# safe-autonomous-systems/fluidgym

Hardware: NVIDIA B200
Metric: env-steps/sec (solver steps x envs) (higher is better)
Workload: dtype f32

## Files before the change

fluidgym_b200/csrc/piso_b200.cu:

```cuda
#include <cuda_runtime.h>
#include <cooperative_groups.h>
#include <stdint.h>
#include <stdio.h>
#include <stdlib.h>
#include <string.h>
#include <math.h>
#include <new>

#include "fluidgym_b200.h"

namespace cg = cooperative_groups;

static thread_local char g_err[512] = "";
static int set_err(int code, const char *msg, cudaError_t ce = cudaSuccess) {
    if (ce != cudaSuccess) snprintf(g_err, sizeof(g_err), "%s: %s", msg, cudaGetErrorString(ce));
    else snprintf(g_err, sizeof(g_err), "%s", msg);
    return code;
}
extern "C" const char *fgb_last_error(void) { return g_err; }
extern "C" int fgb_version(void) { return 1; }

#define LAUNCH_CHECK(name)                                                       \
    do {                                                                         \
        cudaError_t e_ = cudaGetLastError();                                     \
        if (e_ != cudaSuccess) return set_err(FGB_E_CUDA, name, e_);             \
    } while (0)

typedef fgb_tables Tab;

struct fgb_batch {
    Tab t;
    int B;
    fgb_options opt;
    char *ws;
    size_t ws_bytes;
    float *Coff, *A, *rhs, *ures, *Poff, *Pdiag, *hbya, *div, *pres, *kry;
    float *resid, *dt, *maxvel, *fluxbal, *pmean;
    double *remaining;
    int32_t *iters, *active, *nsub, *counters;
    int32_t *h_counters;
    unsigned long long *iter_total;
    long long launches;
    int asm_envs;
    int prof_on;
    static const int PROF_MAX = 8192;
    cudaEvent_t *prof_ev;
    int *prof_cls;
    int prof_n;
    static const int MAX_GROUPS = 8;
    int groups;
    fgb_batch *parent;
    int pmean_stride;
    cudaStream_t gstream[MAX_GROUPS];
    cudaEvent_t gfork, gjoin[MAX_GROUPS];
};
enum { CLS_CG = 0, CLS_BICG = 1, CLS_ASM = 2, CLS_OTHER = 3 };
struct ProfScope {
    fgb_batch *b; cudaStream_t st; int idx;
    ProfScope(fgb_batch *b_, int cls, cudaStream_t st_) : b(b_->parent ? b_->parent : b_), st(st_), idx(-1) {
        b_->launches++;
        if (b->prof_on && b->prof_n < fgb_batch::PROF_MAX) {
            idx = b->prof_n++;
            b->prof_cls[idx] = cls;
            cudaEventRecord(b->prof_ev[2 * idx], st);
        }
    }
    ~ProfScope() { if (idx >= 0) cudaEventRecord(b->prof_ev[2 * idx + 1], st); }
};

static size_t align_up(size_t x) { return (x + 255) & ~(size_t)255; }

struct Carver {
    char *base; size_t off;
    template <typename T> T *take(size_t n) { T *p = (T *)(base + off); off = align_up(off + n * sizeof(T)); return p; }
};
static const int KRY_VECS = 12;
// ... 9 lines not shown
    b->fluxbal = c.take<float>(b->B); b->pmean = c.take<float>(8 * (size_t)b->B); b->remaining = c.take<double>(b->B);
    b->iters = c.take<int32_t>(8 * (size_t)b->B); b->active = c.take<int32_t>(b->B); b->nsub = c.take<int32_t>(b->B);
    b->counters = c.take<int32_t>(64);
    b->iter_total = c.take<unsigned long long>(2 * (size_t)b->B);
    *total = c.off;
}

extern "C" size_t fgb_workspace_bytes(const fgb_tables *t, int32_t B) {
    fgb_batch tmp; memset(&tmp, 0, sizeof(tmp)); tmp.t = *t; tmp.B = B;
    size_t total = 0; carve(&tmp, nullptr, &total);
    return total;
}

static fgb_options default_options() {
    fgb_options o; o.corrector_steps = 2; o.adv_nonortho_steps = 1; o.p_nonortho_steps = 1; o.nonortho = 1;
    o.adv_tol = 1e-5f; o.p_tol = 1e-5f; o.max_iter = 5000; o.cg_impl = 0; return o;
}

extern "C" int fgb_batch_create(const fgb_tables *t, int32_t B, void *workspace, size_t workspace_bytes,
                                const fgb_options *opt, fgb_batch **out) {
    if (!t || !out || B <= 0 || t->N <= 0) return set_err(FGB_E_ARG, "fgb_batch_create: bad argument");
    int ndev = 0;
    cudaError_t ce = cudaGetDeviceCount(&ndev);
    if (ce != cudaSuccess || ndev == 0) return set_err(FGB_E_CUDA, "fgb_batch_create: no CUDA device (there is no CPU fallback)", ce);
    size_t need = fgb_workspace_bytes(t, B);
    if (!workspace || workspace_bytes < need) return set_err(FGB_E_WORKSPACE, "fgb_batch_create: workspace too small");
    fgb_batch *b = new (std::nothrow) fgb_batch();
    if (!b) return set_err(FGB_E_ARG, "fgb_batch_create: out of host memory");
    memset(b, 0, sizeof(*b));
    b->t = *t; b->B = B; b->opt = opt ? *opt : default_options();
    b->ws = (char *)workspace; b->ws_bytes = workspace_bytes;
    b->asm_envs = 1;
    if (const char *ev = getenv("FGB_ASM_ENVS")) { const int v = atoi(ev); if (v == 2 || v == 4 || v == 8) b->asm_envs = v; }
    b->groups = 1; b->pmean_stride = B;
    if (const char *ev = getenv("FGB_GROUPS")) { const int v = atoi(ev); if (v >= 1 && v <= fgb_batch::MAX_GROUPS) b->groups = v; }
    size_t total; carve(b, b->ws, &total);
    ce = cudaMallocHost(&b->h_counters, 64 * sizeof(int32_t));
    if (ce != cudaSuccess) { delete b; return set_err(FGB_E_CUDA, "cudaMallocHost", ce); }
    ce = cudaMemset(b->ws, 0, need);
    if (ce != cudaSuccess) { cudaFreeHost(b->h_counters); delete b; return set_err(FGB_E_CUDA, "cudaMemset workspace", ce); }
    *out = b;
    return FGB_OK;
}
extern "C" int fgb_batch_set_groups(fgb_batch *b, int32_t groups) {
    if (!b || groups < 1 || groups > fgb_batch::MAX_GROUPS) return set_err(FGB_E_ARG, "fgb_batch_set_groups: 1 <= groups <= 8");
    b->groups = groups;
    return FGB_OK;
}
extern "C" void fgb_batch_destroy(fgb_batch *b) {
    if (!b) return;
    if (b->gfork) {
        cudaEventDestroy(b->gfork);
        for (int g = 0; g < fgb_batch::MAX_GROUPS; ++g) { cudaEventDestroy(b->gjoin[g]); cudaStreamDestroy(b->gstream[g]); }
    }
    if (b->h_counters) cudaFreeHost(b->h_counters);
    if (b->prof_ev) { for (int i = 0; i < 2 * fgb_batch::PROF_MAX; ++i) cudaEventDestroy(b->prof_ev[i]); delete[] b->prof_ev; delete[] b->prof_cls; }
    delete b;
}
extern "C" int fgb_profile_enable(fgb_batch *b, int on) {
    if (!b) return set_err(FGB_E_ARG, "fgb_profile_enable: null argument");
    if (on && !b->prof_ev) {
        b->prof_ev = new cudaEvent_t[2 * fgb_batch::PROF_MAX];
        b->prof_cls = new int[fgb_batch::PROF_MAX];
        for (int i = 0; i < 2 * fgb_batch::PROF_MAX; ++i) {
            cudaError_t ce = cudaEventCreate(&b->prof_ev[i]);
            if (ce != cudaSuccess) return set_err(FGB_E_CUDA, "cudaEventCreate", ce);
// ... 138 lines not shown
        face_fluxes(t, g, u, bv, nb, fl);
        float diag = det / dt + t.Cd[g];
        float *co = Coff + (size_t)b * 4 * N;
#pragma unroll
        for (int f = 0; f < 4; ++f) {
            float o = 0.f;
            if (nb[f] >= 0) {
                const float ff = ((f & 1) ? 0.5f : -0.5f) * fl[f];
                diag += ff;
                o = (ff + t.Cd[(f + 1) * N + g]) / det;
            }
            co[f * N + g] = o;
        }
        A[(size_t)b * N + g] = diag / det;
    }
    float S[2];
    boundary_source(t, bv, nb, S);
    float no0 = 0.f, no1 = 0.f;
    for (int k = 0; k < t.K_no; ++k) {
        const float w = t.no_wv[k * N + g];
        if (w != 0.f) { const int j = t.no_idx[k * N + g]; no0 += w * ur[j]; no1 += w * ur[N + j]; }
    }
    for (int k = 0; k < t.K_nob; ++k) {
        const float w = t.nob_w[k * N + g];
        if (w != 0.f) { const int j = t.nob_idx[k * N + g]; no0 += w * bv[j]; no1 += w * bv[NB + j]; }
    }
    float r0 = (det * u[g] / dt + S[0] - no0) / det;
    float r1 = (det * u[N + g] / dt + S[1] - no1) / det;
    if (Src) { r0 += Src[(size_t)b * 2 * N + g]; r1 += Src[(size_t)b * 2 * N + N + g]; }
    Rhs[(size_t)b * 2 * N + g] = r0;
    Rhs[(size_t)b * 2 * N + N + g] = r1;
}

__global__ void __launch_bounds__(256) k_setup_pressure_matrix(Tab t, const float *__restrict__ A, const int32_t *__restrict__ active,
                                                                float *__restrict__ Poff, float *__restrict__ Pdiag) {
    const int b = blockIdx.y;
    if (active && !active[b]) return;
    const int g = blockIdx.x * blockDim.x + threadIdx.x;
    const int N = t.N;
    if (g >= N) return;
    const float *a = A + (size_t)b * N;
    float rA[5];
    rA[0] = 1.0f / a[g];
#pragma unroll
    for (int f = 0; f < 4; ++f) { const int nb = t.nbr[f * N + g]; rA[f + 1] = nb >= 0 ? 1.0f / a[nb] : rA[0]; }
    float P[5];
#pragma unroll
    for (int e = 0; e < 5; ++e) {
        float s = 0.f;
#pragma unroll
        for (int j = 0; j < 5; ++j) s += t.Wp[(5 * e + j) * N + g] * rA[j];
        P[e] = s;
    }
    Pdiag[(size_t)b * N + g] = P[0];
#pragma unroll
    for (int f = 0; f < 4; ++f) Poff[(size_t)b * 4 * N + f * N + g] = P[f + 1];
}

__global__ void __launch_bounds__(256) k_hbya(Tab t, const float *__restrict__ U, const float *__restrict__ Ures,
                                               const float *__restrict__ Bvel, const float *__restrict__ Src,
                                               const float *__restrict__ Coff, const float *__restrict__ A,
                                               const float *__restrict__ dtv, const int32_t *__restrict__ active,
                                               float *__restrict__ Hbya) {
    const int b = blockIdx.y;
    if (active && !active[b]) return;
    const int g = blockIdx.x * blockDim.x + threadIdx.x;
    const int N = t.N, NB = t.NB;
    if (g >= N) return;
    const float *u = U + (size_t)b * 2 * N, *ur = Ures + (size_t)b * 2 * N, *bv = Bvel + (size_t)b * 2 * NB;
    const float *co = Coff + (size_t)b * 4 * N;
    const float dt = dtv[b];
    int nb[4];
#pragma unroll
    for (int f = 0; f < 4; ++f) nb[f] = t.nbr[f * N + g];
    float H0 = 0.f, H1 = 0.f;
#pragma unroll
    for (int f = 0; f < 4; ++f)
        if (nb[f] >= 0) { const float c = co[f * N + g]; H0 += c * ur[nb[f]]; H1 += c * ur[N + nb[f]]; }
    float S[2];
    boundary_source(t, bv, nb, S);
    const float det = t.det[g];
    float s0 = S[0] / det, s1 = S[1] / det;
    if (Src) { s0 += Src[(size_t)b * 2 * N + g]; s1 += Src[(size_t)b * 2 * N + N + g]; }
    const float rD = 1.0f / A[(size_t)b * N + g];
    Hbya[(size_t)b * 2 * N + g] = rD * (u[g] / dt - H0 + s0);
    Hbya[(size_t)b * 2 * N + N + g] = rD * (u[N + g] / dt - H1 + s1);
}

__global__ void __launch_bounds__(256) k_pressure_div(Tab t, const float *__restrict__ Hbya, const float *__restrict__ Bvel,
                                                       const float *__restrict__ Pprev, const float *__restrict__ A,
                                                       const int32_t *__restrict__ active, int nonortho, float *__restrict__ Div) {
    const int b = blockIdx.y;
    if (active && !active[b]) return;
    const int g = blockIdx.x * blockDim.x + threadIdx.x;
    const int N = t.N, NB = t.NB;
    if (g >= N) return;
    const float *h = Hbya + (size_t)b * 2 * N, *bv = Bvel + (size_t)b * 2 * NB;
    int nb[4];
#pragma unroll
    for (int f = 0; f < 4; ++f) nb[f] = t.nbr[f * N + g];
    float fl[4];
    face_fluxes(t, g, h, bv, nb, fl);
    float d = (fl[1] - fl[0]) + (fl[3] - fl[2]);
    if (nonortho) {
        const float *a = A + (size_t)b * N, *pp = Pprev + (size_t)b * N;
        float rA[5];
        rA[0] = 1.0f / a[g];
#pragma unroll
        for (int f = 0; f < 4; ++f) rA[f + 1] = nb[f] >= 0 ? 1.0f / a[nb[f]] : rA[0];
        float S = 0.f;
        for (int k = 0; k < t.K_no; ++k) {
            const float gP = t.no_gP[k * N + g], gN = t.no_gN[k * N + g];
            if (gP != 0.f || gN != 0.f) {
                const int fc = t.no_face[k * N + g];
                const float rn = fc == 0 ? rA[1] : fc == 1 ? rA[2] : fc == 2 ? rA[3] : rA[4];
                S += (gP * rA[0] + gN * rn) * pp[t.no_idx[k * N + g]];
            }
        }
        d += S;
    }
    Div[(size_t)b * N + g] = d;
}

template <int E>
__global__ void __launch_bounds__(256) k_setup_pressure_matrix_multi(Tab t, int B, const float *__restrict__ A,
                                                                      const int32_t *__restrict__ active, float *__restrict__ Poff,
                                                                      float *__restrict__ Pdiag) {
    const int b0 = blockIdx.y * E;
    const int g = blockIdx.x * blockDim.x + threadIdx.x;
    const int N = t.N;
    if (g >= N) return;
    int nb[4];
#pragma unroll
    for (int f = 0; f < 4; ++f) nb[f] = t.nbr[f * N + g];
    float W[25];
#pragma unroll
    for (int q = 0; q < 25; ++q) W[q] = t.Wp[q * N + g];
    float P[E][5];
    bool on[E];
#pragma unroll
    for (int e = 0; e < E; ++e) {
        const int b = b0 + e;
        on[e] = b < B && !(active && !active[b]);
        if (!on[e]) continue;
        const float *a = A + (size_t)b * N;
        float rA[5];
        rA[0] = 1.0f / a[g];
#pragma unroll
        for (int f = 0; f < 4; ++f) rA[f + 1] = nb[f] >= 0 ? 1.0f / a[nb[f]] : rA[0];
#pragma unroll
        for (int q = 0; q < 5; ++q) {
            float sacc = 0.f;
#pragma unroll
            for (int j = 0; j < 5; ++j) sacc += W[5 * q + j] * rA[j];
// ... 170 lines not shown
                if (on[e]) { const float *ur = Ures + (size_t)(b0 + e) * 2 * N; no0[e] += w * ur[j]; no1[e] += w * ur[N + j]; }
        }
    }
    for (int k = 0; k < t.K_nob; ++k) {
        const float w = t.nob_w[k * N + g];
        if (w != 0.f) {
            const int j = t.nob_idx[k * N + g];
#pragma unroll
            for (int e = 0; e < E; ++e)
                if (on[e]) { const float *bv = Bvel + (size_t)(b0 + e) * 2 * NB; no0[e] += w * bv[j]; no1[e] += w * bv[NB + j]; }
        }
    }
#pragma unroll
    for (int e = 0; e < E; ++e) {
        if (!on[e]) continue;
        const int b = b0 + e;
        const float *u = U + (size_t)b * 2 * N;
        float r0 = (det * u[g] / dt[e] + S0[e] - no0[e]) / det;
        float r1 = (det * u[N + g] / dt[e] + S1[e] - no1[e]) / det;
        if (Src) { r0 += Src[(size_t)b * 2 * N + g]; r1 += Src[(size_t)b * 2 * N + N + g]; }
        Rhs[(size_t)b * 2 * N + g] = r0;
        Rhs[(size_t)b * 2 * N + N + g] = r1;
    }
}

__global__ void __launch_bounds__(256) k_correct_velocity(Tab t, const float *__restrict__ Hbya, const float *__restrict__ P,
                                                           const float *__restrict__ A, const int32_t *__restrict__ active,
                                                           float *__restrict__ Uout) {
    const int b = blockIdx.y;
    if (active && !active[b]) return;
    const int g = blockIdx.x * blockDim.x + threadIdx.x;
    const int N = t.N;
    if (g >= N) return;
    const float *p = P + (size_t)b * N;
    const float pc = p[g];
    float pg[2];
#pragma unroll
    for (int d = 0; d < 2; ++d) {
        const int nl = t.nbr[(2 * d) * N + g], nu = t.nbr[(2 * d + 1) * N + g];
        const float fac = (nl < 0 || nu < 0) ? 1.0f : 0.5f;
        const float vl = nl >= 0 ? p[nl] : pc, vu = nu >= 0 ? p[nu] : pc;
        pg[d] = (vu - vl) * fac;
    }
    const float gx = pg[0] * t.minv[g] + pg[1] * t.minv[2 * N + g];
    const float gy = pg[0] * t.minv[N + g] + pg[1] * t.minv[3 * N + g];
    const float rD = 1.0f / A[(size_t)b * N + g];
    Uout[(size_t)b * 2 * N + g] = -rD * gx + Hbya[(size_t)b * 2 * N + g];
    Uout[(size_t)b * 2 * N + N + g] = -rD * gy + Hbya[(size_t)b * 2 * N + N + g];
}

__global__ void __launch_bounds__(256) k_setup_scalar(Tab t, const float *__restrict__ U, const float *__restrict__ Tin,
                                                       const float *__restrict__ Bvel, const float *__restrict__ Sbval,
                                                       const float *__restrict__ dtv, const int32_t *__restrict__ active,
                                                       float *__restrict__ Coff, float *__restrict__ A, float *__restrict__ Rhs) {
    const int b = blockIdx.y;
    if (active && !active[b]) return;
    const int g = blockIdx.x * blockDim.x + threadIdx.x;
    const int N = t.N, NB = t.NB;
    if (g >= N) return;
    const float *u = U + (size_t)b * 2 * N, *bv = Bvel + (size_t)b * 2 * NB, *sb = Sbval + (size_t)b * NB;
    const float dt = dtv[b];
    const float det = t.det[g];
    int nb[4];
#pragma unroll
    for (int f = 0; f < 4; ++f) nb[f] = t.nbr[f * N + g];
    float fl[4];
    face_fluxes(t, g, u, bv, nb, fl);
    float diag = det / dt + t.Cd_s[g];
    float r = det * Tin[(size_t)b * N + g] / dt;
    float *co = Coff + (size_t)b * 4 * N;
#pragma unroll
    for (int f = 0; f < 4; ++f) {
        float o = 0.f;
        if (nb[f] >= 0) {
            const float ff = ((f & 1) ? 0.5f : -0.5f) * fl[f];
            diag += ff;
            o = (ff + t.Cd_s[(f + 1) * N + g]) / det;
        } else {
            const int j = -1 - nb[f];
            const float sc = sb[j];
            const float flux = fl[f] * ((f & 1) ? 1.f : -1.f);
// ... 671 lines not shown
#pragma unroll
                    for (int k = 0; k < CPT; ++k) bs[threadIdx.x + k * T] = xr[k];
                }
                if (i > 0 && crit >= lastc) ++rising; else rising = 0;
                lastc = crit;
                if (crit < tol) stop = 1;
                else if (i == maxit - 1 || rising >= 100) stop = 2;
            }
            asm volatile("" : "+r"(stop));
            if (stop) { take_best = stop == 2; break; }
            const float beta = rr2 / rho;
            rho = rr2;
#pragma unroll
            for (int k = 0; k < CPT; ++k) vs[threadIdx.x + k * T] = rr[k] + beta * pk[k];
            publish();
        }
        if (take_best) {
#pragma unroll
            for (int k = 0; k < CPT; ++k) xr[k] = bs[threadIdx.x + k * T];
            used = best_it; fin = bestc;
        }
    }
    float sx = 0.f;
#pragma unroll
    for (int k = 0; k < CPT; ++k) sx += xr[k];
    const float mean = (flags & 2) ? 0.f : cluster_sum(sx) / (float)N;
    if (mean_out && threadIdx.x == 0 && rank == 0) mean_out[b] = mean;
#pragma unroll
    for (int k = 0; k < CPT; ++k) { const int l = threadIdx.x + k * T; if (l < cnt) xo[start + l] = xr[k] - mean; }
    if (threadIdx.x == 0 && rank == 0) { iters[b * 8 + 2 + slot] = used; resid[b * 8 + 2 + slot] = fin; iter_total[b * 2] += (unsigned long long)(used + 1); }
    cluster_sync_all();
}

template <int T, int CPT, int CS, int MINB>
__global__ void __launch_bounds__(T, MINB) k_cg_strip(Tab t, const float *__restrict__ Poff, const float *__restrict__ Pdiag,
                                                    const float *__restrict__ Rhs, float *__restrict__ Xout,
                                                    int maxit, float tol, int zero_init, int reset_steps, int slot,
                                                    const int32_t *__restrict__ active, int32_t *__restrict__ iters,
                                                    float *__restrict__ resid, unsigned long long *__restrict__ iter_total,
                                                    int flags, float *__restrict__ mean_out, float *__restrict__ best) {
    static_assert(T % 32 == 0, "whole warps only: every warp contributes exactly one partial sum per exchange");
    constexpr int NW = T / 32;
    const int b = blockIdx.x / CS;
    uint32_t rank;
    asm volatile("mov.u32 %0, %%cluster_ctarank;" : "=r"(rank));
    if (active && !active[b]) return;
    extern __shared__ __align__(16) float smem[];
    const int N = t.N, SL = t.st_slots, G = t.st_gmax;
    float4 *co4 = reinterpret_cast<float4 *>(smem);
    float *cdg = smem + 4 * CPT * T;
    float *vs = cdg + CPT * T;
    float *rs = vs + SL;
    float *red = rs + G;
    float *wpart = red + 2 * CS + (2 * CS & 1 ? 1 : 0);
    unsigned long long *mb = (unsigned long long *)(wpart + 2 * NW + (2 * NW & 1 ? 1 : 0));
    uint2 *rex = (uint2 *)(mb + 4);
    uint2 *lex = rex + t.st_remax;
    const float *off = Poff + (size_t)b * 4 * N, *dg = Pdiag + (size_t)b * N, *f = Rhs + (size_t)b * N;
    float *xo = Xout + (size_t)b * N;
    const float norm = 1.0f / sqrtf((float)N);
    const uint32_t red_addr = smem_u32(red), mb_addr = smem_u32(mb), rs_addr = smem_u32(rs);
    const int tid = threadIdx.x, lane = tid & 31, warp = tid >> 5;

    const int4 th0 = reinterpret_cast<const int4 *>(t.st_thread)[((size_t)rank * T + tid) * 2];
    const int4 th1 = reinterpret_cast<const int4 *>(t.st_thread)[((size_t)rank * T + tid) * 2 + 1];
    const int S = th0.y;
    float *vp = vs + th0.x;
    const int re_off = th0.w & 0xffff, re_cnt = (th0.w >> 16) & 0xff;
    const int n_lex = t.st_cnt[4 * rank + 2];
    const float *rgp = rs + th1.y;
    const uint32_t rm = (uint32_t)th1.z;
    const int32_t *cellp = t.st_cell + ((size_t)rank * T + tid) * CPT;
    float *bestp = best + ((size_t)b * CS + rank) * T * CPT + tid;
    const uint32_t bytesA = CS * 4u, bytesB = CS * 4u + 4u * (uint32_t)t.st_cnt[4 * rank];
    if (tid == 0) {
        mbar_init(mb_addr, 1); mbar_init(mb_addr + 8, 1);
        mbar_init(mb_addr + 16, NW); mbar_init(mb_addr + 24, NW);
        asm volatile("fence.mbarrier_init.release.cluster;" ::: "memory");
        mbar_arrive_expect_tx(mb_addr, bytesA);
        mbar_arrive_expect_tx(mb_addr + 8, bytesB);
    }
    for (int e = tid; e < t.st_cnt[4 * rank + 1]; e += T) {
        const int32_t a = t.st_rexp[((size_t)rank * t.st_remax + e) * 2], d = t.st_rexp[((size_t)rank * t.st_remax + e) * 2 + 1];
        rex[e] = make_uint2((uint32_t)a, mapa_u32(rs_addr + 4u * (uint32_t)d, (uint32_t)a >> 8));
    }
    for (int e = tid; e < n_lex; e += T)
        lex[e] = make_uint2((uint32_t)t.st_lexp[((size_t)rank * t.st_lemax + e) * 2], (uint32_t)t.st_lexp[((size_t)rank * t.st_lemax + e) * 2 + 1]);
    for (int i = tid; i < SL + G; i += T) vs[i] = 0.f;

    float x[CPT], r[CPT], ap[CPT];
#pragma unroll
    for (int k = 0; k < CPT; ++k) {
        const int c = cellp[k];
        const bool real = c >= 0;
        const int g = real ? c : (c <= -2 ? -2 - c : 0);
        float co[4];
#pragma unroll
        for (int d = 0; d < 4; ++d) {
            const int ff = (th0.z >> (2 * d)) & 3;
            const int nb = real ? t.nbr[ff * N + g] : -1;
            if (flags & 1) co[d] = nb >= 0 ? off[(int)t.rev[ff * N + g] * N + nb] : 0.f;
            else co[d] = nb >= 0 ? off[ff * N + g] : 0.f;
        }
        co4[k * T + tid] = make_float4(co[0], co[1], co[2], co[3]);
        cdg[k * T + tid] = real ? dg[g] : 0.f;
        x[k] = (c != -1 && !zero_init) ? xo[g] : 0.f;
        r[k] = real ? f[g] : 0.f;
        ap[k] = 0.f;
    }
    const uint32_t peer_red = mapa_u32(red_addr, (uint32_t)(lane < CS ? lane : 0));
    const uint32_t peer_mb = mapa_u32(mb_addr, (uint32_t)(lane < CS ? lane : 0));
    cluster_sync_all();

    uint32_t parA = 0, parB = 0;
    auto exchange = [&](float a0, const uint32_t which, uint32_t &par, const uint32_t bytes) -> float {
#pragma unroll
        for (int o = 16; o > 0; o >>= 1) a0 += __shfl_xor_sync(0xffffffffu, a0, o);
        if (lane == 0) {
            wpart[which * NW + warp] = a0;
            asm volatile("mbarrier.arrive.release.cta.shared::cta.b64 _, [%0];" ::"r"(mb_addr + 16u + 8u * which) : "memory");
        }
        if (warp == 0) {
            mbar_wait_sleep(mb_addr + 16u + 8u * which, par);
            float s1 = lane < NW ? wpart[which * NW + lane] : 0.f;
#pragma unroll
            for (int o = 16; o > 0; o >>= 1) s1 += __shfl_xor_sync(0xffffffffu, s1, o);
            if (lane < CS) st_async_f32(peer_red + 4u * (which * CS + rank), s1, peer_mb + 8u * which);
        }
        mbar_wait_sleep(mb_addr + 8u * which, par); par ^= 1u;
        float s0 = 0.f;
#pragma unroll
        for (int q = 0; q < CS; ++q) s0 += red[which * CS + q];
        if (tid == 0) mbar_arrive_expect_tx(mb_addr + 8u * which, bytes);
        return s0;
    };
    auto row_of = [&](const float (&v)[CPT], int kk) -> float {
        float s = v[0];
#pragma unroll
        for (int k = 1; k < CPT; ++k) s = (kk == k) ? v[k] : s;
        return s;
    };
// ... 25 lines not shown
    };
    auto publish_x = [&]() {
#pragma unroll
        for (int k = 0; k < CPT; ++k) vp[k * S] = x[k];
        mirror_local_ghosts();
    };
    auto new_direction = [&](float beta) {
        if (rm) {
            int n = 0;
#pragma unroll
            for (int k = 0; k < CPT; ++k) if (rm & (1u << k)) r[k] = rgp[n++];
        }
#pragma unroll
        for (int k = 0; k < CPT; ++k) ap[k] = vp[k * S];
#pragma unroll
        for (int k = 0; k < CPT; ++k) vp[k * S] = fmaf(beta, ap[k], r[k]);
        if (rm) {
#pragma unroll
            for (int k = 0; k < CPT; ++k) if (rm & (1u << k)) r[k] = 0.f;
        }
        mirror_local_ghosts();
    };
    auto residual_norm2 = [&]() -> float {
        for (int j = 0; j < re_cnt; ++j) {
            const uint2 ex = rex[re_off + j];
            st_async_f32(ex.y, row_of(r, (int)(ex.x & 0xff)), mapa_u32(mb_addr + 8, ex.x >> 8));
        }
        float a0 = 0.f, a1 = 0.f;
#pragma unroll
        for (int k = 0; k < CPT; k += 2) { a0 = fmaf(r[k], r[k], a0); if (k + 1 < CPT) a1 = fmaf(r[k + 1], r[k + 1], a1); }
        return exchange(a0 + a1, 1u, parB, bytesB);
    };

    float nz = 0.f;
#pragma unroll
    for (int k = 0; k < CPT; ++k) nz += (r[k] != 0.f) ? 1.f : 0.f;
    const float nzt = exchange(nz, 0u, parA, bytesA);
    int used = -1; float fin = 0.f;
    bool solved = false;
    if (!(nzt > 0.f)) {
#pragma unroll
        for (int k = 0; k < CPT; ++k) x[k] = 0.f;
    } else {
        solved = true;
        if (!zero_init) {
            publish_x();
            (void)spmv();
#pragma unroll
            for (int k = 0; k < CPT; ++k) r[k] -= ap[k];
            __syncthreads();
        }
#pragma unroll
        for (int k = 0; k < CPT; ++k) bestp[k * T] = x[k];
        float rho = residual_norm2();
        new_direction(0.f);
        float bestc = 0.f, lastc = 0.f; int best_it = -1, rising = 0;
        bool take_best = false;
        int until_reset = reset_steps > 0 ? reset_steps - 1 : -1;
        for (int i = 0; i < maxit; ++i) {
            if (until_reset == 0) {
                until_reset = reset_steps;
                (void)exchange(0.f, 0u, parA, bytesA);
                publish_x();
                (void)spmv();
#pragma unroll
                for (int k = 0; k < CPT; ++k) { const int c = cellp[k]; r[k] = (c >= 0 ? f[c] : 0.f) - ap[k]; }
// ... 17 lines not shown
                if (i == 0 || crit < bestc) {
                    bestc = crit; best_it = i;
#pragma unroll
                    for (int k = 0; k < CPT; ++k) bestp[k * T] = x[k];
                }
                if (i > 0 && crit >= lastc) ++rising; else rising = 0;
                lastc = crit;
                if (crit < tol) stop = 1;
                else if (i == maxit - 1 || rising >= 100) stop = 2;
            }
            asm volatile("" : "+r"(stop));
            if (stop) { take_best = stop == 2; break; }
            const float beta = rr2 / rho;
            rho = rr2;
            new_direction(beta);
        }
        if (take_best) {
#pragma unroll
            for (int k = 0; k < CPT; ++k) x[k] = bestp[k * T];
            used = best_it; fin = bestc;
        }
    }
    float mean = 0.f;
    if (solved && !(flags & 2)) {
        float sx = 0.f;
#pragma unroll
        for (int k = 0; k < CPT; ++k) sx += (cellp[k] >= 0) ? x[k] : 0.f;
        mean = exchange(sx, 0u, parA, bytesA) / (float)N;
    }
    if (mean_out && tid == 0 && rank == 0) mean_out[b] = mean;
#pragma unroll
    for (int k = 0; k < CPT; ++k) { const int c = cellp[k]; if (c >= 0) xo[c] = x[k] - mean; }
    if (tid == 0 && rank == 0) { iters[b * 8 + 2 + slot] = used; resid[b * 8 + 2 + slot] = fin; iter_total[b * 2] += (unsigned long long)(used + 1); }
    cluster_sync_all();
}

template <int E> struct EnvTag { static constexpr int value = E; };

template <int T, int CPT, int CS>
__global__ void __launch_bounds__(T, 1) k_cg_strip2(Tab t, const float *__restrict__ Poff, const float *__restrict__ Pdiag,
                                                    const float *__restrict__ Rhs, float *__restrict__ Xout, int B,
                                                    int maxit, float tol, int zero_init, int reset_steps, int slot,
                                                    const int32_t *__restrict__ active, int32_t *__restrict__ iters,
                                                    float *__restrict__ resid, unsigned long long *__restrict__ iter_total,
                                                    int flags, float *__restrict__ mean_out, float *__restrict__ best) {
    static_assert(T % 32 == 0, "whole warps only");
    constexpr int NW = T / 32;
    constexpr uint32_t FULL = 0xffffffffu;
    const int b0 = 2 * (int)(blockIdx.x / CS);
    uint32_t rank;
    asm volatile("mov.u32 %0, %%cluster_ctarank;" : "=r"(rank));
    bool on[2];
    on[0] = !active || active[b0];
    on[1] = b0 + 1 < B && (!active || active[b0 + 1]);
    if (!on[0] && !on[1]) return;
    extern __shared__ __align__(16) float smem[];
    const int N = t.N, SL = t.st_slots, G = t.st_gmax;
    const int ENVF = (5 * CPT * T + SL + G + 2 * CS + 2 * NW + 3) & ~3;
    unsigned long long *mb = (unsigned long long *)(smem + 2 * ENVF);
    unsigned int *cnt = (unsigned int *)(mb + 4);
    uint2 *rex = (uint2 *)(cnt + 4);
    uint2 *lex = rex + t.st_remax;
    const float norm = 1.0f / sqrtf((float)N);
    const uint32_t mb_addr = smem_u32(mb);
    const int tid = threadIdx.x, lane = tid & 31, warp = tid >> 5;

    const int4 th0 = reinterpret_cast<const int4 *>(t.st_thread)[((size_t)rank * T + tid) * 2];
// ... 1541 lines not shown
    }
    cudaLaunchConfig_t cfg; memset(&cfg, 0, sizeof(cfg));
    cfg.gridDim = dim3(b->B * CS); cfg.blockDim = dim3(T); cfg.dynamicSmemBytes = smem; cfg.stream = st;
    cudaLaunchAttribute attr[1];
    attr[0].id = cudaLaunchAttributeClusterDimension;
    attr[0].val.clusterDim.x = CS; attr[0].val.clusterDim.y = 1; attr[0].val.clusterDim.z = 1;
    cfg.attrs = attr; cfg.numAttrs = 1;
    ce = cudaLaunchKernelEx(&cfg, kern, b->t, poff, pdiag, rhs, p_out, max_iter, b->opt.p_tol, zero_init, reset_steps, slot, active,
                            b->iters, b->resid, b->iter_total, flags, mean_out, b->kry);
    if (ce != cudaSuccess) return set_err(FGB_E_CUDA, "cudaLaunchKernelEx(k_cg_strip)", ce);
    return FGB_OK;
}

template <int T, int CPT, int MINB>
static int cg_strip_cs(fgb_batch *b, const float *poff, const float *pdiag, const float *rhs, float *p_out, int zero_init,
                       int reset_steps, int max_iter, int slot, const int32_t *active, int flags, float *mean_out, cudaStream_t st) {
    int rc = launch_cg_strip<T, CPT, 1, MINB>(b, poff, pdiag, rhs, p_out, zero_init, reset_steps, max_iter, slot, active, flags, mean_out, st);
    if (rc == 1) rc = launch_cg_strip<T, CPT, 2, MINB>(b, poff, pdiag, rhs, p_out, zero_init, reset_steps, max_iter, slot, active, flags, mean_out, st);
    if (rc == 1) rc = launch_cg_strip<T, CPT, 4, MINB>(b, poff, pdiag, rhs, p_out, zero_init, reset_steps, max_iter, slot, active, flags, mean_out, st);
    if (rc == 1) rc = launch_cg_strip<T, CPT, 8, MINB>(b, poff, pdiag, rhs, p_out, zero_init, reset_steps, max_iter, slot, active, flags, mean_out, st);
    if (rc == 1) rc = launch_cg_strip<T, CPT, 16, MINB>(b, poff, pdiag, rhs, p_out, zero_init, reset_steps, max_iter, slot, active, flags, mean_out, st);
    return rc;
}
static int cg_strip_any(fgb_batch *b, const float *poff, const float *pdiag, const float *rhs, float *p_out, int zero_init,
                        int reset_steps, int max_iter, int slot, const int32_t *active, int flags, float *mean_out, cudaStream_t st) {
    int rc = cg_strip_cs<480, 17, 1>(b, poff, pdiag, rhs, p_out, zero_init, reset_steps, max_iter, slot, active, flags, mean_out, st);
    if (rc == 1) rc = cg_strip_cs<256, 17, 2>(b, poff, pdiag, rhs, p_out, zero_init, reset_steps, max_iter, slot, active, flags, mean_out, st);
    if (rc == 1) rc = cg_strip_cs<896, 9, 1>(b, poff, pdiag, rhs, p_out, zero_init, reset_steps, max_iter, slot, active, flags, mean_out, st);
    if (rc == 1) rc = cg_strip_cs<640, 13, 1>(b, poff, pdiag, rhs, p_out, zero_init, reset_steps, max_iter, slot, active, flags, mean_out, st);
    if (rc == 1) rc = cg_strip_cs<320, 13, 2>(b, poff, pdiag, rhs, p_out, zero_init, reset_steps, max_iter, slot, active, flags, mean_out, st);
    return rc;
}


template <int T, int CPT, int CS>
static int launch_cg_strip2(fgb_batch *b, const float *poff, const float *pdiag, const float *rhs, float *p_out, int zero_init,
                            int reset_steps, int max_iter, int slot, const int32_t *active, int flags, float *mean_out,
                            cudaStream_t st) {
    if (b->t.st_cs != CS || b->t.st_T != T || b->t.st_cpt != CPT) return 1;
    if ((size_t)CS * T * CPT > (size_t)KRY_VECS * b->t.N)
        return set_err(FGB_E_ARG, "cg_impl 12: domain too small for the best-iterate scratch (use cg_impl 6)");
    const size_t envf = ((size_t)5 * CPT * T + (size_t)b->t.st_slots + (size_t)b->t.st_gmax + (size_t)2 * CS + 2 * (T / 32) + 3) & ~(size_t)3;
    const size_t smem = 2 * envf * sizeof(float) + 4 * 8 + 4 * 4 + ((size_t)b->t.st_remax + (size_t)b->t.st_lemax) * 8;
    if (smem > 227 * 1024 || (b->t.st_slots & 3) || (b->t.st_gmax & 1))
        return set_err(FGB_E_ARG, "cg_impl 12: strip plan does not fit in shared memory");
    auto kern = k_cg_strip2<T, CPT, CS>;
    cudaError_t ce = cudaFuncSetAttribute(kern, cudaFuncAttributeMaxDynamicSharedMemorySize, (int)smem);
    if (ce != cudaSuccess) return set_err(FGB_E_CUDA, "cudaFuncSetAttribute(k_cg_strip2)", ce);
    if (CS > 8) {
        ce = cudaFuncSetAttribute(kern, cudaFuncAttributeNonPortableClusterSizeAllowed, 1);
        if (ce != cudaSuccess) return set_err(FGB_E_CUDA, "cudaFuncSetAttribute(k_cg_strip2, non-portable cluster)", ce);
    }
    cudaLaunchConfig_t cfg; memset(&cfg, 0, sizeof(cfg));
    cfg.gridDim = dim3(((b->B + 1) / 2) * CS); cfg.blockDim = dim3(T); cfg.dynamicSmemBytes = smem; cfg.stream = st;
    cudaLaunchAttribute attr[1];
    attr[0].id = cudaLaunchAttributeClusterDimension;
    attr[0].val.clusterDim.x = CS; attr[0].val.clusterDim.y = 1; attr[0].val.clusterDim.z = 1;
    cfg.attrs = attr; cfg.numAttrs = 1;
    ce = cudaLaunchKernelEx(&cfg, kern, b->t, poff, pdiag, rhs, p_out, b->B, max_iter, b->opt.p_tol, zero_init, reset_steps, slot, active,
                            b->iters, b->resid, b->iter_total, flags, mean_out, b->kry);
    if (ce != cudaSuccess) return set_err(FGB_E_CUDA, "cudaLaunchKernelEx(k_cg_strip2)", ce);
    return FGB_OK;
}
static int cg_strip2_any(fgb_batch *b, const float *poff, const float *pdiag, const float *rhs, float *p_out, int zero_init,
                         int reset_steps, int max_iter, int slot, const int32_t *active, int flags, float *mean_out, cudaStream_t st) {
    int rc = launch_cg_strip2<480, 9, 2>(b, poff, pdiag, rhs, p_out, zero_init, reset_steps, max_iter, slot, active, flags, mean_out, st);
// ... 168 lines not shown
static int piso_substep_impl(fgb_batch *b, float *u, float *p, const float *bvel, const float *src, const float *dt,
                             const int32_t *active, const fgb_scalar *sc, fgb_stream_t s) {
    int rc;
    const fgb_options &o = b->opt;
    cudaStream_t st = STREAM(s);
    const int N = b->t.N;
    if (sc) {
        if (!sc->T || !sc->sbval || !sc->src || !b->t.Cd_s || !b->t.sb_neumann)
            return set_err(FGB_E_ARG, "fgb_piso_substep: incomplete scalar description / tables");
        {
            ProfScope ps(b, CLS_ASM, st);
            k_setup_scalar<<<cell_grid(b), 256, 0, st>>>(b->t, u, sc->T, bvel, sc->sbval, dt, active, b->Coff, b->A, b->rhs);
            LAUNCH_CHECK("k_setup_scalar");
        }
        {
            ProfScope ps(b, CLS_BICG, st);
            if ((rc = run_bicgstab<1>(b, b->rhs, sc->T, 1, active, st))) return rc;
        }
        b->launches++;
        k_buoyancy<<<cell_grid(b), 256, 0, st>>>(sc->T, sc->beta, N, active, sc->src);
        LAUNCH_CHECK("k_buoyancy");
        src = sc->src;
    }
    const int n_adv = o.nonortho ? o.adv_nonortho_steps : 1;
    for (int ns = 0; ns < n_adv; ++ns) {
        b->launches++;
        launch_setup_advection(b, st, u, ns == 0 ? u : b->ures, bvel, src, dt, active, ns == 0);
        LAUNCH_CHECK("k_setup_advection");
        if ((rc = fgb_solve_advection(b, o.nonortho ? (ns == 0) : 0, active, s))) return rc;
    }
    int slot = 0;
    const int n_p = o.nonortho ? o.p_nonortho_steps : 1;
    const int reset = o.nonortho ? 100 : 0;
    for (int cs = 0; cs < o.corrector_steps; ++cs) {
        if (cs == 0) { if ((rc = fgb_setup_pressure_matrix(b, active, s))) return rc; }
        for (int ps = 0; ps < n_p; ++ps) {
            if ((rc = fgb_setup_pressure_rhs(b, u, bvel, src, p, dt, ps == 0, active, s))) return rc;
            if ((rc = solve_pressure_slot(b, p, ps == 0, reset, o.max_iter, slot++, active, s))) return rc;
        }
        if ((rc = fgb_correct_velocity(b, p, b->ures, active, s))) return rc;
    }
    b->launches++;
    k_copy_active<<<dim3((2 * N + 255) / 256, b->B), 256, 0, st>>>(b->ures, u, 2 * N, active);
    LAUNCH_CHECK("k_copy_active");
    return FGB_OK;
}

static int copy_async(void *dst, const void *src, size_t bytes, cudaStream_t st) {
    cudaError_t ce = cudaMemcpyAsync(dst, src, bytes, cudaMemcpyDeviceToDevice, st);
    return ce == cudaSuccess ? FGB_OK : set_err(FGB_E_CUDA, "cudaMemcpyAsync (tape)", ce);
}

static int record_impl(fgb_batch *b, float *u, float *p, const float *bvel, const float *dt, const fgb_tape *tp,
                       const fgb_scalar *sc, const fgb_tape_scalar *stp, fgb_stream_t s) {
    const fgb_options &o = b->opt;
    const int C = o.corrector_steps, n_adv = o.nonortho ? o.adv_nonortho_steps : 1, n_p = o.nonortho ? o.p_nonortho_steps : 1;
    const int reset = 0;
    if ((o.cg_impl != 3 && !uses_halo_plan(o.cg_impl) && o.cg_impl != 7 && o.cg_impl != 8) || C < 1 || n_adv < 1 || n_p < 1 || C * n_p > 8)
        return set_err(FGB_E_ARG, "fgb_piso_substep_record: needs cg_impl 3 or 6 and correctors x pressure iterations <= 8");
    cudaStream_t st = STREAM(s);
    const size_t B = b->B, N = b->t.N, NB = b->t.NB;
    const int32_t *act = tp->active;
    int rc;
    if ((rc = copy_async(tp->u_in, u, 2 * B * N * 4, st))) return rc;
    if ((rc = copy_async(tp->p_in, p, B * N * 4, st))) return rc;
    if ((rc = copy_async(tp->bvel_in, bvel, 2 * B * NB * 4, st))) return rc;
// ... 364 lines not shown
```

Before: 48380.

## Fuse PISO corrector stages into a single cluster CG kernel

New measurement: 35450 (median of 6 runs). 0.733x the previous value.

```diff
diff --git a/fluidgym_b200/csrc/piso_b200.cu b/fluidgym_b200/csrc/piso_b200.cu
--- a/fluidgym_b200/csrc/piso_b200.cu
+++ b/fluidgym_b200/csrc/piso_b200.cu
@@ -42,6 +42,7 @@
     unsigned long long *iter_total;
     long long launches;
     int asm_envs;
+    int fused_stages;
     int prof_on;
     static const int PROF_MAX = 8192;
     cudaEvent_t *prof_ev;
@@ -117,6 +118,8 @@
     b->ws = (char *)workspace; b->ws_bytes = workspace_bytes;
     b->asm_envs = 1;
     if (const char *ev = getenv("FGB_ASM_ENVS")) { const int v = atoi(ev); if (v == 2 || v == 4 || v == 8) b->asm_envs = v; }
+    b->fused_stages = 1;
+    if (const char *ev = getenv("FGB_FUSED_STAGES")) b->fused_stages = atoi(ev) != 0;
     b->groups = 1; b->pmean_stride = B;
     if (const char *ev = getenv("FGB_GROUPS")) { const int v = atoi(ev); if (v >= 1 && v <= fgb_batch::MAX_GROUPS) b->groups = v; }
     size_t total; carve(b, b->ws, &total);
@@ -321,6 +324,87 @@
     Rhs[(size_t)b * 2 * N + N + g] = r1;
 }
 
+__device__ __forceinline__ void pressure_matrix_row(const Tab &t, const float *a, int g, float P[5]) {
+    const int N = t.N;
+    float rA[5];
+    rA[0] = 1.0f / a[g];
+#pragma unroll
+    for (int f = 0; f < 4; ++f) { const int nb = t.nbr[f * N + g]; rA[f + 1] = nb >= 0 ? 1.0f / a[nb] : rA[0]; }
+#pragma unroll
+    for (int e = 0; e < 5; ++e) {
+        float s = 0.f;
+#pragma unroll
+        for (int j = 0; j < 5; ++j) s += t.Wp[(5 * e + j) * N + g] * rA[j];
+        P[e] = s;
+    }
+}
+
+__device__ __forceinline__ void hbya_cell(const Tab &t, int g, const float *u, const float *ur, const float *bv, const float *src,
+                                          const float *co, const float *a, float dt, float H[2]) {
+    const int N = t.N;
+    int nb[4];
+#pragma unroll
+    for (int f = 0; f < 4; ++f) nb[f] = t.nbr[f * N + g];
+    float H0 = 0.f, H1 = 0.f;
+#pragma unroll
+    for (int f = 0; f < 4; ++f)
+        if (nb[f] >= 0) { const float c = co[f * N + g]; H0 += c * ur[nb[f]]; H1 += c * ur[N + nb[f]]; }
+    float S[2];
+    boundary_source(t, bv, nb, S);
+    const float det = t.det[g];
+    float s0 = S[0] / det, s1 = S[1] / det;
+    if (src) { s0 += src[g]; s1 += src[N + g]; }
+    const float rD = 1.0f / a[g];
+    H[0] = rD * (u[g] / dt - H0 + s0);
+    H[1] = rD * (u[N + g] / dt - H1 + s1);
+}
+
+__device__ __forceinline__ float pressure_div_cell(const Tab &t, int g, const float *h, const float *bv, const float *pp, const float *a,
+                                                   int nonortho) {
+    const int N = t.N;
+    int nb[4];
+#pragma unroll
+    for (int f = 0; f < 4; ++f) nb[f] = t.nbr[f * N + g];
+    float fl[4];
+    face_fluxes(t, g, h, bv, nb, fl);
+    float d = (fl[1] - fl[0]) + (fl[3] - fl[2]);
+    if (nonortho) {
+        float rA[5];
+        rA[0] = 1.0f / a[g];
+#pragma unroll
+        for (int f = 0; f < 4; ++f) rA[f + 1] = nb[f] >= 0 ? 1.0f / a[nb[f]] : rA[0];
+        float S = 0.f;
+        for (int k = 0; k < t.K_no; ++k) {
+            const float gP = t.no_gP[k * N + g], gN = t.no_gN[k * N + g];
+            if (gP != 0.f || gN != 0.f) {
+                const int fc = t.no_face[k * N + g];
+                const float rn = fc == 0 ? rA[1] : fc == 1 ? rA[2] : fc == 2 ? rA[3] : rA[4];
+                S += (gP * rA[0] + gN * rn) * pp[t.no_idx[k * N + g]];
+            }
+        }
+        d += S;
+    }
+    return d;
+}
+
+__device__ __forceinline__ void correct_velocity_cell(const Tab &t, int g, const float *p, const float *hb, const float *a, float U[2]) {
+    const int N = t.N;
+    const float pc = p[g];
+    float pg[2];
+#pragma unroll
+    for (int d = 0; d < 2; ++d) {
+        const int nl = t.nbr[(2 * d) * N + g], nu = t.nbr[(2 * d + 1) * N + g];
+        const float fac = (nl < 0 || nu < 0) ? 1.0f : 0.5f;
+        const float vl = nl >= 0 ? p[nl] : pc, vu = nu >= 0 ? p[nu] : pc;
+        pg[d] = (vu - vl) * fac;
+    }
+    const float gx = pg[0] * t.minv[g] + pg[1] * t.minv[2 * N + g];
+    const float gy = pg[0] * t.minv[N + g] + pg[1] * t.minv[3 * N + g];
+    const float rD = 1.0f / a[g];
+    U[0] = -rD * gx + hb[g];
+    U[1] = -rD * gy + hb[N + g];
+}
+
 __global__ void __launch_bounds__(256) k_setup_pressure_matrix(Tab t, const float *__restrict__ A, const int32_t *__restrict__ active,
                                                                 float *__restrict__ Poff, float *__restrict__ Pdiag) {
     const int b = blockIdx.y;
@@ -328,19 +412,8 @@
     const int g = blockIdx.x * blockDim.x + threadIdx.x;
     const int N = t.N;
     if (g >= N) return;
-    const float *a = A + (size_t)b * N;
-    float rA[5];
-    rA[0] = 1.0f / a[g];
-#pragma unroll
-    for (int f = 0; f < 4; ++f) { const int nb = t.nbr[f * N + g]; rA[f + 1] = nb >= 0 ? 1.0f / a[nb] : rA[0]; }
     float P[5];
-#pragma unroll
-    for (int e = 0; e < 5; ++e) {
-        float s = 0.f;
-#pragma unroll
-        for (int j = 0; j < 5; ++j) s += t.Wp[(5 * e + j) * N + g] * rA[j];
-        P[e] = s;
-    }
+    pressure_matrix_row(t, A + (size_t)b * N, g, P);
     Pdiag[(size_t)b * N + g] = P[0];
 #pragma unroll
     for (int f = 0; f < 4; ++f) Poff[(size_t)b * 4 * N + f * N + g] = P[f + 1];
@@ -356,24 +429,11 @@
     const int g = blockIdx.x * blockDim.x + threadIdx.x;
     const int N = t.N, NB = t.NB;
     if (g >= N) return;
-    const float *u = U + (size_t)b * 2 * N, *ur = Ures + (size_t)b * 2 * N, *bv = Bvel + (size_t)b * 2 * NB;
-    const float *co = Coff + (size_t)b * 4 * N;
-    const float dt = dtv[b];
-    int nb[4];
-#pragma unroll
-    for (int f = 0; f < 4; ++f) nb[f] = t.nbr[f * N + g];
-    float H0 = 0.f, H1 = 0.f;
-#pragma unroll
-    for (int f = 0; f < 4; ++f)
-        if (nb[f] >= 0) { const float c = co[f * N + g]; H0 += c * ur[nb[f]]; H1 += c * ur[N + nb[f]]; }
-    float S[2];
-    boundary_source(t, bv, nb, S);
-    const float det = t.det[g];
-    float s0 = S[0] / det, s1 = S[1] / det;
-    if (Src) { s0 += Src[(size_t)b * 2 * N + g]; s1 += Src[(size_t)b * 2 * N + N + g]; }
-    const float rD = 1.0f / A[(size_t)b * N + g];
-    Hbya[(size_t)b * 2 * N + g] = rD * (u[g] / dt - H0 + s0);
-    Hbya[(size_t)b * 2 * N + N + g] = rD * (u[N + g] / dt - H1 + s1);
+    float H[2];
+    hbya_cell(t, g, U + (size_t)b * 2 * N, Ures + (size_t)b * 2 * N, Bvel + (size_t)b * 2 * NB, Src ? Src + (size_t)b * 2 * N : nullptr,
+              Coff + (size_t)b * 4 * N, A + (size_t)b * N, dtv[b], H);
+    Hbya[(size_t)b * 2 * N + g] = H[0];
+    Hbya[(size_t)b * 2 * N + N + g] = H[1];
 }
 
 __global__ void __launch_bounds__(256) k_pressure_div(Tab t, const float *__restrict__ Hbya, const float *__restrict__ Bvel,
@@ -384,31 +444,8 @@
     const int g = blockIdx.x * blockDim.x + threadIdx.x;
     const int N = t.N, NB = t.NB;
     if (g >= N) return;
-    const float *h = Hbya + (size_t)b * 2 * N, *bv = Bvel + (size_t)b * 2 * NB;
-    int nb[4];
-#pragma unroll
-    for (int f = 0; f < 4; ++f) nb[f] = t.nbr[f * N + g];
-    float fl[4];
-    face_fluxes(t, g, h, bv, nb, fl);
-    float d = (fl[1] - fl[0]) + (fl[3] - fl[2]);
-    if (nonortho) {
-        const float *a = A + (size_t)b * N, *pp = Pprev + (size_t)b * N;
-        float rA[5];
-        rA[0] = 1.0f / a[g];
-#pragma unroll
-        for (int f = 0; f < 4; ++f) rA[f + 1] = nb[f] >= 0 ? 1.0f / a[nb[f]] : rA[0];
-        float S = 0.f;
-        for (int k = 0; k < t.K_no; ++k) {
-            const float gP = t.no_gP[k * N + g], gN = t.no_gN[k * N + g];
-            if (gP != 0.f || gN != 0.f) {
-                const int fc = t.no_face[k * N + g];
-                const float rn = fc == 0 ? rA[1] : fc == 1 ? rA[2] : fc == 2 ? rA[3] : rA[4];
-                S += (gP * rA[0] + gN * rn) * pp[t.no_idx[k * N + g]];
-            }
-        }
-        d += S;
-    }
-    Div[(size_t)b * N + g] = d;
+    Div[(size_t)b * N + g] = pressure_div_cell(t, g, Hbya + (size_t)b * 2 * N, Bvel + (size_t)b * 2 * NB,
+                                               nonortho ? Pprev + (size_t)b * N : nullptr, A + (size_t)b * N, nonortho);
 }
 
 template <int E>
@@ -645,21 +682,10 @@
     const int g = blockIdx.x * blockDim.x + threadIdx.x;
     const int N = t.N;
     if (g >= N) return;
-    const float *p = P + (size_t)b * N;
-    const float pc = p[g];
-    float pg[2];
-#pragma unroll
-    for (int d = 0; d < 2; ++d) {
-        const int nl = t.nbr[(2 * d) * N + g], nu = t.nbr[(2 * d + 1) * N + g];
-        const float fac = (nl < 0 || nu < 0) ? 1.0f : 0.5f;
-        const float vl = nl >= 0 ? p[nl] : pc, vu = nu >= 0 ? p[nu] : pc;
-        pg[d] = (vu - vl) * fac;
-    }
-    const float gx = pg[0] * t.minv[g] + pg[1] * t.minv[2 * N + g];
-    const float gy = pg[0] * t.minv[N + g] + pg[1] * t.minv[3 * N + g];
-    const float rD = 1.0f / A[(size_t)b * N + g];
-    Uout[(size_t)b * 2 * N + g] = -rD * gx + Hbya[(size_t)b * 2 * N + g];
-    Uout[(size_t)b * 2 * N + N + g] = -rD * gy + Hbya[(size_t)b * 2 * N + N + g];
+    float U[2];
+    correct_velocity_cell(t, g, P + (size_t)b * N, Hbya + (size_t)b * 2 * N, A + (size_t)b * N, U);
+    Uout[(size_t)b * 2 * N + g] = U[0];
+    Uout[(size_t)b * 2 * N + N + g] = U[1];
 }
 
 __global__ void __launch_bounds__(256) k_setup_scalar(Tab t, const float *__restrict__ U, const float *__restrict__ Tin,
@@ -1397,13 +1423,36 @@
     cluster_sync_all();
 }
 
-template <int T, int CPT, int CS, int MINB>
-__global__ void __launch_bounds__(T, MINB) k_cg_strip(Tab t, const float *__restrict__ Poff, const float *__restrict__ Pdiag,
-                                                    const float *__restrict__ Rhs, float *__restrict__ Xout,
-                                                    int maxit, float tol, int zero_init, int reset_steps, int slot,
-                                                    const int32_t *__restrict__ active, int32_t *__restrict__ iters,
-                                                    float *__restrict__ resid, unsigned long long *__restrict__ iter_total,
-                                                    int flags, float *__restrict__ mean_out, float *__restrict__ best) {
+template <int U, int W, class Cell, class Store>
+__device__ __forceinline__ void strided_cells(int first, int stride, int N, Cell cell, Store store) {
+    for (int g0 = first; g0 < N; g0 += U * stride) {
+        float v[U][W];
+#pragma unroll
+        for (int j = 0; j < U; ++j) if (g0 + j * stride < N) cell(g0 + j * stride, v[j]);
+#pragma unroll
+        for (int j = 0; j < U; ++j) if (g0 + j * stride < N) store(g0 + j * stride, v[j]);
+    }
+}
+
+#ifndef FGB_PHASE_CELLS
+#define FGB_PHASE_CELLS 4
+#endif
+#ifndef FGB_MAT_CELLS
+#define FGB_MAT_CELLS 2
+#endif
+constexpr int PHASE_CELLS = FGB_PHASE_CELLS, MAT_CELLS = FGB_MAT_CELLS;
+
+struct CorrectorArgs {
+    float *u, *ures, *p, *Poff, *Pdiag, *hbya, *div, *pmean;
+    const float *bvel, *src, *dt, *A, *Coff;
+    int corrector_steps, p_steps, nonortho, pmean_stride;
+};
+
+template <int T, int CPT, int CS, bool FUSED>
+__device__ __forceinline__ void cg_strip_body(const Tab &t, const float *Poff, const float *Pdiag, const float *Rhs, float *Xout,
+                                              int maxit, float tol, int zero_init, int reset_steps, int slot,
+                                              const int32_t *active, int32_t *iters, float *resid, unsigned long long *iter_total,
+                                              int flags, float *mean_out, float *best, const CorrectorArgs &ca) {
     static_assert(T % 32 == 0, "whole warps only: every warp contributes exactly one partial sum per exchange");
     constexpr int NW = T / 32;
     const int b = blockIdx.x / CS;
@@ -1452,6 +1501,17 @@
     for (int e = tid; e < n_lex; e += T)
         lex[e] = make_uint2((uint32_t)t.st_lexp[((size_t)rank * t.st_lemax + e) * 2], (uint32_t)t.st_lexp[((size_t)rank * t.st_lemax + e) * 2 + 1]);
     for (int i = tid; i < SL + G; i += T) vs[i] = 0.f;
+    if constexpr (FUSED) {
+        const float *a = ca.A + (size_t)b * N;
+        float *po = ca.Poff + (size_t)b * 4 * N, *pd = ca.Pdiag + (size_t)b * N;
+        strided_cells<MAT_CELLS, 5>(rank * T + tid, CS * T, N, [&](int g, float (&P)[5]) { pressure_matrix_row(t, a, g, P); },
+                                      [&](int g, const float (&P)[5]) {
+                                          pd[g] = P[0];
+#pragma unroll
+                                          for (int e = 0; e < 4; ++e) po[e * N + g] = P[e + 1];
+                                      });
+        cluster_sync_all();
+    }
 
     float x[CPT], r[CPT], ap[CPT];
 #pragma unroll
@@ -1469,9 +1529,11 @@
         }
         co4[k * T + tid] = make_float4(co[0], co[1], co[2], co[3]);
         cdg[k * T + tid] = real ? dg[g] : 0.f;
-        x[k] = (c != -1 && !zero_init) ? xo[g] : 0.f;
-        r[k] = real ? f[g] : 0.f;
-        ap[k] = 0.f;
+        if constexpr (!FUSED) {
+            x[k] = (c != -1 && !zero_init) ? xo[g] : 0.f;
+            r[k] = real ? f[g] : 0.f;
+            ap[k] = 0.f;
+        }
     }
     const uint32_t peer_red = mapa_u32(red_addr, (uint32_t)(lane < CS ? lane : 0));
     const uint32_t peer_mb = mapa_u32(mb_addr, (uint32_t)(lane < CS ? lane : 0));
@@ -1563,6 +1625,41 @@
         return exchange(a0 + a1, 1u, parB, bytesB);
     };
 
+    const int n_pass = FUSED ? ca.corrector_steps * ca.p_steps : 1;
+    for (int pass = 0; pass < n_pass; ++pass) {
+    if constexpr (FUSED) {
+        const int ps = pass % ca.p_steps;
+        zero_init = ps == 0;
+        mean_out = ca.pmean + (size_t)(pass > 7 ? 7 : pass) * ca.pmean_stride;
+        slot = pass > 5 ? 5 : pass;
+        const size_t N2 = 2 * (size_t)N * b;
+        const float *bv = ca.bvel + (size_t)b * 2 * t.NB;
+        const float *a = ca.A + (size_t)b * N;
+        float *hb = ca.hbya + N2;
+        if (ps == 0) {
+            const float dt = ca.dt[b];
+            const float *u = ca.u + N2, *ur = ca.ures + N2, *src = ca.src ? ca.src + N2 : nullptr, *co = ca.Coff + (size_t)b * 4 * N;
+            strided_cells<PHASE_CELLS, 2>(rank * T + tid, CS * T, N, [&](int g, float (&H)[2]) { hbya_cell(t, g, u, ur, bv, src, co, a, dt, H); },
+                                          [&](int g, const float (&H)[2]) { hb[g] = H[0]; hb[N + g] = H[1]; });
+            cluster_sync_all();
+        }
+        {
+            const float *pp = ca.p + (size_t)b * N;
+            float *dv = ca.div + (size_t)b * N;
+            strided_cells<PHASE_CELLS, 1>(rank * T + tid, CS * T, N,
+                                          [&](int g, float (&d)[1]) { d[0] = pressure_div_cell(t, g, hb, bv, pp, a, ca.nonortho); },
+                                          [&](int g, const float (&d)[1]) { dv[g] = d[0]; });
+        }
+        cluster_sync_all();
+#pragma unroll
+        for (int k = 0; k < CPT; ++k) {
+            const int c = cellp[k];
+            const int g = c >= 0 ? c : (c <= -2 ? -2 - c : 0);
+            x[k] = (c != -1 && !zero_init) ? xo[g] : 0.f;
+            r[k] = c >= 0 ? f[g] : 0.f;
+            ap[k] = 0.f;
+        }
+    }
     float nz = 0.f;
 #pragma unroll
     for (int k = 0; k < CPT; ++k) nz += (r[k] != 0.f) ? 1.f : 0.f;
@@ -1646,7 +1743,44 @@
 #pragma unroll
     for (int k = 0; k < CPT; ++k) { const int c = cellp[k]; if (c >= 0) xo[c] = x[k] - mean; }
     if (tid == 0 && rank == 0) { iters[b * 8 + 2 + slot] = used; resid[b * 8 + 2 + slot] = fin; iter_total[b * 2] += (unsigned long long)(used + 1); }
+    if constexpr (FUSED) {
+        if (pass + 1 < n_pass) cluster_sync_all();
+        if (pass % ca.p_steps == ca.p_steps - 1) {
+            if (pass + 1 == n_pass) cluster_sync_all();
+            const size_t N2 = 2 * (size_t)N * b;
+            const bool last = pass + 1 == n_pass;
+            const float *pp = ca.p + (size_t)b * N, *hb = ca.hbya + N2, *a = ca.A + (size_t)b * N;
+            float *ur = ca.ures + N2, *u = ca.u + N2;
+            strided_cells<PHASE_CELLS, 2>(rank * T + tid, CS * T, N, [&](int g, float (&U)[2]) { correct_velocity_cell(t, g, pp, hb, a, U); },
+                                          [&](int g, const float (&U)[2]) {
+                                              ur[g] = U[0]; ur[N + g] = U[1];
+                                              if (last) { u[g] = U[0]; u[N + g] = U[1]; }
+                                          });
+            if (pass + 1 < n_pass) cluster_sync_all();
+        }
+    }
+    }
     cluster_sync_all();
+}
+
+template <int T, int CPT, int CS, int MINB>
+__global__ void __launch_bounds__(T, MINB) k_cg_strip(Tab t, const float *__restrict__ Poff, const float *__restrict__ Pdiag,
+                                                    const float *__restrict__ Rhs, float *__restrict__ Xout,
+                                                    int maxit, float tol, int zero_init, int reset_steps, int slot,
+                                                    const int32_t *__restrict__ active, int32_t *__restrict__ iters,
+                                                    float *__restrict__ resid, unsigned long long *__restrict__ iter_total,
+                                                    int flags, float *__restrict__ mean_out, float *__restrict__ best) {
+    cg_strip_body<T, CPT, CS, false>(t, Poff, Pdiag, Rhs, Xout, maxit, tol, zero_init, reset_steps, slot, active, iters, resid, iter_total,
+                                     flags, mean_out, best, CorrectorArgs{});
+}
+
+template <int T, int CPT, int CS, int MINB>
+__global__ void __launch_bounds__(T, MINB) k_piso_corrector(Tab t, CorrectorArgs ca, int maxit, float tol, int reset_steps,
+                                                          const int32_t *__restrict__ active, int32_t *__restrict__ iters,
+                                                          float *__restrict__ resid, unsigned long long *__restrict__ iter_total,
+                                                          float *__restrict__ best) {
+    cg_strip_body<T, CPT, CS, true>(t, ca.Poff, ca.Pdiag, ca.div, ca.p, maxit, tol, 1, reset_steps, 0, active, iters, resid, iter_total,
+                                    0, nullptr, best, ca);
 }
 
 template <int E> struct EnvTag { static constexpr int value = E; };
@@ -3254,6 +3388,40 @@
     return rc;
 }
 
+template <int T, int CPT, int CS, int MINB>
+static int launch_piso_corrector(fgb_batch *b, const CorrectorArgs &ca, int reset_steps, const int32_t *active, cudaStream_t st) {
+    if (b->t.st_cs != CS || b->t.st_T != T || b->t.st_cpt != CPT) return 1;
+    if ((size_t)CS * T * CPT > (size_t)KRY_VECS * b->t.N)
+        return set_err(FGB_E_ARG, "cg_impl 11: domain too small for the best-iterate scratch (use cg_impl 6)");
+    const size_t smem = ((size_t)5 * CPT * T + (size_t)b->t.st_slots + (size_t)b->t.st_gmax + (size_t)2 * CS + 2 * (T / 32) + 2) * sizeof(float) + 4 * 8 +
+                        ((size_t)b->t.st_remax + (size_t)b->t.st_lemax) * 8;
+    if (smem > 227 * 1024 || (b->t.st_slots & 3) || (b->t.st_gmax & 1))
+        return set_err(FGB_E_ARG, "cg_impl 11: strip plan does not fit in shared memory");
+    auto kern = k_piso_corrector<T, CPT, CS, MINB>;
+    cudaError_t ce = cudaFuncSetAttribute(kern, cudaFuncAttributeMaxDynamicSharedMemorySize, (int)smem);
+    if (ce != cudaSuccess) return set_err(FGB_E_CUDA, "cudaFuncSetAttribute(k_piso_corrector)", ce);
+    if (CS > 8) {
+        ce = cudaFuncSetAttribute(kern, cudaFuncAttributeNonPortableClusterSizeAllowed, 1);
+        if (ce != cudaSuccess) return set_err(FGB_E_CUDA, "cudaFuncSetAttribute(k_piso_corrector, non-portable cluster)", ce);
+    }
+    cudaLaunchConfig_t cfg; memset(&cfg, 0, sizeof(cfg));
+    cfg.gridDim = dim3(b->B * CS); cfg.blockDim = dim3(T); cfg.dynamicSmemBytes = smem; cfg.stream = st;
+    cudaLaunchAttribute attr[1];
+    attr[0].id = cudaLaunchAttributeClusterDimension;
+    attr[0].val.clusterDim.x = CS; attr[0].val.clusterDim.y = 1; attr[0].val.clusterDim.z = 1;
+    cfg.attrs = attr; cfg.numAttrs = 1;
+    ce = cudaLaunchKernelEx(&cfg, kern, b->t, ca, b->opt.max_iter, b->opt.p_tol, reset_steps, active, b->iters, b->resid, b->iter_total, b->kry);
+    if (ce != cudaSuccess) return set_err(FGB_E_CUDA, "cudaLaunchKernelEx(k_piso_corrector)", ce);
+    return FGB_OK;
+}
+static int piso_corrector_any(fgb_batch *b, const CorrectorArgs &ca, int reset_steps, const int32_t *active, cudaStream_t st) {
+    int rc = launch_piso_corrector<480, 17, 1, 1>(b, ca, reset_steps, active, st);
+    if (rc == 1) rc = launch_piso_corrector<480, 17, 2, 1>(b, ca, reset_steps, active, st);
+    if (rc == 1) rc = launch_piso_corrector<480, 17, 4, 1>(b, ca, reset_steps, active, st);
+    if (rc == 1) rc = launch_piso_corrector<480, 17, 8, 1>(b, ca, reset_steps, active, st);
+    if (rc == 1) rc = launch_piso_corrector<480, 17, 16, 1>(b, ca, reset_steps, active, st);
+    return rc;
+}
 
 template <int T, int CPT, int CS>
 static int launch_cg_strip2(fgb_batch *b, const float *poff, const float *pdiag, const float *rhs, float *p_out, int zero_init,
@@ -3488,6 +3656,18 @@
     int slot = 0;
     const int n_p = o.nonortho ? o.p_nonortho_steps : 1;
     const int reset = o.nonortho ? 100 : 0;
+    if (b->fused_stages && o.cg_impl == 11 && b->t.st_thread && b->t.st_cell && b->t.st_rexp && b->t.st_lexp && b->t.st_cnt &&
+        b->t.st_T == 480 && b->t.st_cpt == 17 && o.corrector_steps > 0) {
+        CorrectorArgs ca;
+        ca.u = u; ca.ures = b->ures; ca.p = p; ca.Poff = b->Poff; ca.Pdiag = b->Pdiag; ca.hbya = b->hbya; ca.div = b->div; ca.pmean = b->pmean;
+        ca.bvel = bvel; ca.src = src; ca.dt = dt; ca.A = b->A; ca.Coff = b->Coff;
+        ca.corrector_steps = o.corrector_steps; ca.p_steps = n_p; ca.nonortho = o.nonortho; ca.pmean_stride = b->pmean_stride;
+        ProfScope ps(b, CLS_CG, st);
+        rc = piso_corrector_any(b, ca, reset, active, st);
+        if (rc == 1) return set_err(FGB_E_ARG, "fgb_piso_substep: no k_piso_corrector instantiation for the cluster size of this strip plan");
+        if (rc == 0) LAUNCH_CHECK("k_piso_corrector");
+        return rc;
+    }
     for (int cs = 0; cs < o.corrector_steps; ++cs) {
         if (cs == 0) { if ((rc = fgb_setup_pressure_matrix(b, active, s))) return rc; }
         for (int ps = 0; ps < n_p; ++ps) {
```
